# linnanwang/FastGen

Measured on AMD Instinct MI355X. Metric: images/sec at 4-step distilled (DMD2) sampling, higher is better.
Workload: dtype fp32 (tensors, accumulate) with split-bf16 x3 MFMA conv products; 1 GPU; EDM CIFAR-10 32x32 SongUNet (55.7M params) DMD2 4-step 'sde' sampling, batch=512 per GPU; global_batch=512, sample_steps=4, parallelism=replicas x1 (no data-path collective), graph=True

## Files before the change

### fastgen_amd/_lib.py

```python
import ctypes
import os
from ctypes import POINTER, c_char_p, c_double, c_float, c_int, c_int64, c_size_t, c_uint64, c_void_p

_HERE = os.path.dirname(os.path.abspath(__file__))
LIB_PATH = os.path.join(_HERE, "libfastgen_amd.so")

FG_MAX_LEVELS = 8
FG_DTYPE_F32, FG_DTYPE_BF16, FG_DTYPE_BF16X3, FG_DTYPE_FP8 = 0, 1, 2, 3
DTYPE_NAMES = {"fp32": FG_DTYPE_F32, "bf16": FG_DTYPE_BF16, "bf16x3": FG_DTYPE_BF16X3, "fp8": FG_DTYPE_FP8}
FG_SAMPLE_SDE, FG_SAMPLE_ODE = 0, 1
SAMPLE_TYPES = {"sde": FG_SAMPLE_SDE, "ode": FG_SAMPLE_ODE}
FG_LOOP_X0, FG_LOOP_MEANFLOW, FG_LOOP_EULER = 0, 1, 2
LOOP_KINDS = {"x0": FG_LOOP_X0, "meanflow": FG_LOOP_MEANFLOW, "euler": FG_LOOP_EULER}
FG_SCHEDULE_EDM, FG_SCHEDULE_RF = 0, 1
FG_DROP_PRECOND_INPUT, FG_DROP_PRECOND_OUTPUT = 1, 2
FG_BWD_DECODER, FG_BWD_ENCODER, FG_BWD_EMBED = 1, 2, 4
FG_MODEL_SONGUNET, FG_MODEL_DHARIWAL = 0, 1


class fg_edm_config(ctypes.Structure):
    _fields_ = [
        ("img_resolution", c_int), ("img_channels", c_int), ("label_dim", c_int), ("augment_dim", c_int),
        ("model_channels", c_int), ("num_levels", c_int), ("channel_mult", c_int * FG_MAX_LEVELS),
        ("channel_mult_emb", c_int), ("num_blocks", c_int), ("num_attn_resolutions", c_int),
# ... 151 lines not shown
    "fg_wan_bind_param": (c_int, [c_void_p, c_char_p, c_void_p, c_int64]),
    "fg_wan_pack_weights": (c_int, [c_void_p, c_void_p]),
    "fg_wan_pack_group": (c_int, [c_void_p, c_char_p, c_char_p, c_void_p]),
    "fg_wan_workspace_bytes": (c_size_t, [c_void_p, c_int, c_int, c_int, c_int]),
    "fg_wan_clear_caches": (c_int, [c_void_p, c_void_p]),
    "fg_wan_set_text": (c_int, [c_void_p, c_void_p, c_int, c_int, c_void_p, c_size_t, c_void_p]),
    "fg_wan_forward": (c_int, [c_void_p, c_void_p, c_void_p, c_void_p, c_int, c_int, c_int, c_int, c_int, c_int, c_void_p, c_size_t,
                               c_void_p]),
    "fg_wan_forward_block_causal": (c_int, [c_void_p, c_void_p, c_void_p, c_void_p, c_int, c_int, c_int, c_int, c_void_p, c_size_t, c_void_p]),
    "fg_wan_forward_features": (c_int, [c_void_p, c_void_p, c_void_p, c_void_p, c_int, c_int, c_int, c_int, c_int, c_int, c_int, POINTER(c_int),
                                        POINTER(fg_wan_block_taps), c_int, c_void_p, c_void_p, c_void_p, c_size_t, c_void_p]),
    "fg_disc_edm_num_params": (c_int, [c_int]),
    "fg_disc_edm_workspace_bytes": (c_size_t, [c_int, c_int]),
    "fg_disc_edm_run": (c_int, [c_void_p, c_int, c_void_p, c_void_p, c_void_p, c_void_p, c_void_p, c_int, c_void_p, c_size_t, c_void_p]),
    "fg_edm_jvp": (c_int, [c_void_p, c_void_p, c_void_p, c_void_p, c_void_p, c_void_p, c_void_p, c_void_p, c_void_p, c_void_p, c_int,
                           c_void_p, c_size_t, c_void_p]),
    "fg_edm_set_dropout": (c_int, [c_void_p, c_float, c_uint64]),
    "fg_op_dropout_mask": (c_int, [c_void_p, c_int64, c_float, ctypes.c_uint32, c_uint64, c_void_p]),
    "fg_edm_set_augment": (c_int, [c_void_p, c_void_p]),
    "fg_edm_set_training": (c_int, [c_void_p, c_int]),
    "fg_op_images_to_u8": (c_int, [c_void_p, c_void_p, c_int64, c_int, c_int, c_int, c_void_p]),
    "fg_op_randn": (c_int, [c_void_p, c_int64, c_uint64, c_uint64, c_void_p]),
    "fg_op_attention": (c_int, [c_void_p, c_void_p, c_void_p, c_void_p, c_int, c_int, c_int, c_int, c_int, c_void_p]),
    "fg_op_attention_split": (c_int, [c_void_p, c_void_p, c_void_p, c_void_p, c_int, c_int, c_int, c_int, c_int, c_int, c_void_p]),
    "fg_op_attention_plan": (c_int, [c_int, c_int, c_int, c_int, c_int, c_int, c_int, c_int, c_int, POINTER(fg_attention_plan)]),
    "fg_op_attention_ex": (c_int, [c_void_p, c_int, c_int64, c_void_p, c_void_p, c_int, c_int64, c_void_p, c_int, c_int64, c_int, c_int, c_int,
                                   c_int, c_int, c_int, c_int, c_int, c_void_p]),
    "fg_op_gemm_bf16": (c_int, [c_void_p, c_void_p, c_void_p, c_void_p, c_int, c_int, c_int, c_int, c_void_p, c_int, c_int, c_void_p,
                                c_int, c_void_p]),
    "fg_op_quant_rows_fp8": (c_int, [c_int, c_void_p, c_void_p, c_void_p, c_int64, c_int, c_void_p]),
    "fg_op_gemm_fp8": (c_int, [c_void_p, c_void_p, c_void_p, c_void_p, c_int, c_int, c_int, c_int, c_void_p, c_int, c_int, c_void_p,
                               c_int, c_void_p, c_void_p, c_void_p]),
    "fg_op_dit_ln_modulate_fp8": (c_int, [c_void_p, c_void_p, c_int, c_int, c_int, c_void_p, c_void_p, c_int, c_int, c_int, c_void_p]),
    "fg_op_gemm_x3": (c_int, [c_void_p, c_void_p, c_void_p, c_void_p, c_int, c_int, c_int, c_int, c_void_p, c_int, c_int, c_void_p,
                              c_int, c_void_p]),
}

_lib = None


def lib():
    global _lib
    if _lib is None:
        if not os.path.exists(LIB_PATH):
            raise RuntimeError(
                f"{LIB_PATH} not found: build it with `python -c 'import __graft_entry__ as g; g.build()'` "
# ... 19 lines not shown
```

### fastgen_amd/csrc/attn.hip

```cpp
#include <cstdlib>
#include "common.h"
#include "misc.h"

namespace {

template <typename T>
struct PFrag;
template <>
struct PFrag<__bf16> {
    static __device__ __forceinline__ Frag8<__bf16> make(const f32x16& p, int s) {
        Frag8<__bf16> f;
#pragma unroll
        for (int j = 0; j < 8; ++j) f.v[j] = (__bf16)p[8 * s + j];
        return f;
    }
};
template <>
struct PFrag<float> {
    static __device__ __forceinline__ Frag8<float> make(const f32x16& p, int s) {
        Frag8<float> f;
        f.lo = f32x4{p[8 * s + 0], p[8 * s + 1], p[8 * s + 2], p[8 * s + 3]};
        f.hi = f32x4{p[8 * s + 4], p[8 * s + 5], p[8 * s + 6], p[8 * s + 7]};
        return f;
    }
// ... 257 lines not shown
                        mma16(o[d], pf[t * 2 + sub][s2], vf);
                    }
            __syncthreads();
            __builtin_amdgcn_sched_barrier(0);
        }
#pragma unroll
        for (int d = 0; d < 4; ++d)
#pragma unroll
            for (int i = 0; i < 16; ++i) obase[(size_t)acc_row(i, h) * D + (dg * 4 + d) * 32] = (__bf16)o[d][i];
    }
}

constexpr int X3_KP = 272, X3_VP = 136;
constexpr int X3_PLANE = 64 * X3_KP;
constexpr int X3_BUF = 2 * X3_PLANE;

struct AttnMerge {
    const float2* ab;
    const float* bp;
    float2* stats;
    float scale;
};

template <bool MRG>
__global__ __launch_bounds__(256, 2) void attention_x3_lds_kernel(const float* __restrict__ q, const float* __restrict__ k,
                                                                  const float* __restrict__ vt, float* __restrict__ out, int B,
                                                                  AttnMerge mg) {
    constexpr int Tn = 256, D = 256;
    extern __shared__ __attribute__((aligned(16))) char smem[];
    const int tid = threadIdx.x, lane = tid & 63, wave = tid >> 6;
    const int r = lane & 31, h = lane >> 5;
    const int n = blockIdx.x >> 1;
    const int q0 = (blockIdx.x & 1) * 128 + wave * 32;

    auto stage_k = [&](int s, char* buf) {
        const float* src = k + ((size_t)n * Tn + (s & 3) * 64) * D + (s >> 2) * 128;
        f32x4 cf[4];
        if constexpr (MRG) {
            const f32x4* cp = reinterpret_cast<const f32x4*>(mg.ab + (size_t)n * D + (s >> 2) * 128 + (tid & 15) * 8);
#pragma unroll
            for (int j = 0; j < 4; ++j) cf[j] = cp[j];
        }
#pragma unroll
        for (int b2 = 0; b2 < 2; ++b2) {
#pragma unroll
            for (int i = b2 * 2; i < b2 * 2 + 2; ++i) {
                const int idx = tid + 256 * i, row = idx >> 4, c = idx & 15;
                float x[8];
                widen8(load_frag(src + (size_t)row * D + c * 8), x);
                if constexpr (MRG) {
#pragma unroll
                    for (int j = 0; j < 8; ++j) x[j] = fmaf(x[j], cf[j >> 1][2 * (j & 1)], cf[j >> 1][2 * (j & 1) + 1]);
                }
                bf16x8 hi, lo;
                split8(x, hi, lo);
                *reinterpret_cast<bf16x8*>(buf + row * X3_KP + c * 16) = hi;
// ... 4 lines not shown
    };
    auto stage_v = [&](int s, char* buf) {
        const float* src = vt + ((size_t)n * D + (s >> 2) * 128) * Tn + (s & 3) * 64;
#pragma unroll
        for (int b2 = 0; b2 < 2; ++b2) {
#pragma unroll
            for (int i = b2 * 2; i < b2 * 2 + 2; ++i) {
                const int idx = tid + 256 * i, row = idx >> 3, c = idx & 7;
                float x[8];
                widen8(load_frag(src + (size_t)row * Tn + c * 8), x);
                bf16x8 hi, lo;
                split8(x, hi, lo);
                bf16x4* dh = reinterpret_cast<bf16x4*>(buf + row * X3_VP + c * 16);
                dh[0] = bf16x4{hi[0], hi[1], hi[2], hi[3]};
                dh[1] = bf16x4{hi[4], hi[5], hi[6], hi[7]};
                bf16x4* dl = reinterpret_cast<bf16x4*>(buf + X3_PLANE + row * X3_VP + c * 16);
                dl[0] = bf16x4{lo[0], lo[1], lo[2], lo[3]};
                dl[1] = bf16x4{lo[4], lo[5], lo[6], lo[7]};
            }
            __builtin_amdgcn_sched_barrier(0);
        }
    };

    const float* qrow = q + ((size_t)n * Tn + q0 + r) * D + 8 * h;
    f32x16 st[8];
#pragma unroll
    for (int kt = 0; kt < 8; ++kt)
#pragma unroll
        for (int i = 0; i < 16; ++i) st[kt][i] = 0.f;

    stage_k(0, smem);
    __syncthreads();
    Frag8<bf16x3> qf[8];
#pragma unroll
    for (int s = 0; s < 8; ++s) {
        const char* cur = smem + (s & 1) * X3_BUF;
        if ((s & 3) == 0) {
#pragma unroll
            for (int kk = 0; kk < 8; ++kk) qf[kk] = load_op<bf16x3>(qrow + (s >> 2) * 128 + kk * 16);
        }
        if (s + 1 < 8) stage_k(s + 1, smem + ((s + 1) & 1) * X3_BUF);
#pragma unroll
        for (int kk = 0; kk < 8; ++kk) {
#pragma unroll
            for (int sub = 0; sub < 2; ++sub) {
                const char* p = cur + (sub * 32 + r) * X3_KP + (kk * 16 + 8 * h) * 2;
                Frag8<bf16x3> kf;
                kf.hi = *reinterpret_cast<const bf16x8*>(p);
                kf.lo = *reinterpret_cast<const bf16x8*>(p + X3_PLANE);
                mma16(st[(s & 3) * 2 + sub], kf, qf[kk]);
            }
        }
        __syncthreads();
        __builtin_amdgcn_sched_barrier(0);
    }

    float m = -INFINITY;
#pragma unroll
    for (int kt = 0; kt < 8; ++kt)
#pragma unroll
        for (int i = 0; i < 16; ++i) m = fmaxf(m, st[kt][i]);
    m = fmaxf(m, __shfl_xor(m, 32));
    float sum = 0.f;
#pragma unroll
    for (int kt = 0; kt < 8; ++kt)
#pragma unroll
        for (int i = 0; i < 16; ++i) {
            const float e = __builtin_amdgcn_exp2f(1.44269504088896341f * 0.0625f * (st[kt][i] - m));
            st[kt][i] = e;
            sum += e;
        }
    sum += __shfl_xor(sum, 32);
    const float inv = __builtin_amdgcn_rcpf(sum);
    Frag8<bf16x3> pf[8][2];
#pragma unroll
    for (int kt = 0; kt < 8; ++kt) {
#pragma unroll
        for (int s2 = 0; s2 < 2; ++s2) {
            float v[8];
#pragma unroll
            for (int j = 0; j < 8; ++j) v[j] = st[kt][8 * s2 + j] * inv;
            split8(v, pf[kt][s2].hi, pf[kt][s2].lo);
        }
        __builtin_amdgcn_sched_barrier(0);
    }

    float* obase = out + ((size_t)n * Tn + q0) * D + r;
    stage_v(0, smem);
    __syncthreads();
    f32x16 o[4];
#pragma unroll
    for (int s = 0; s < 8; ++s) {
        const char* cur = smem + (s & 1) * X3_BUF;
        if ((s & 3) == 0) {
#pragma unroll
            for (int d = 0; d < 4; ++d)
#pragma unroll
                for (int i = 0; i < 16; ++i) o[d][i] = 0.f;
        }
        if (s + 1 < 8) stage_v(s + 1, smem + ((s + 1) & 1) * X3_BUF);
#pragma unroll
        for (int sub = 0; sub < 2; ++sub)
#pragma unroll
            for (int s2 = 0; s2 < 2; ++s2)
#pragma unroll
                for (int d = 0; d < 4; ++d) {
                    const char* p = cur + (d * 32 + r) * X3_VP + (sub * 32 + 16 * s2 + 4 * h) * 2;
                    const bf16x4 a0 = *reinterpret_cast<const bf16x4*>(p), a1 = *reinterpret_cast<const bf16x4*>(p + 16);
                    const bf16x4 b0 = *reinterpret_cast<const bf16x4*>(p + X3_PLANE), b1 = *reinterpret_cast<const bf16x4*>(p + X3_PLANE + 16);
                    Frag8<bf16x3> vf;
                    vf.hi = bf16x8{a0[0], a0[1], a0[2], a0[3], a1[0], a1[1], a1[2], a1[3]};
                    vf.lo = bf16x8{b0[0], b0[1], b0[2], b0[3], b1[0], b1[1], b1[2], b1[3]};
                    mma16(o[d], pf[(s & 3) * 2 + sub][s2], vf);
                }
        __syncthreads();
        __builtin_amdgcn_sched_barrier(0);
        if ((s & 3) == 3) {
            if constexpr (MRG) {
                const float* xbase = k + ((size_t)n * Tn + q0) * D + r;
#pragma unroll
                for (int d = 0; d < 4; ++d) {
                    const int col = ((s >> 2) * 4 + d) * 32;
                    const float bias = mg.bp[col + r];
                    float sv = 0.f, qv = 0.f;
#pragma unroll
                    for (int i = 0; i < 16; ++i) {
                        const size_t off = (size_t)acc_row(i, h) * D + col;
                        const float v = (o[d][i] + bias + xbase[off]) * mg.scale;
                        obase[off] = v;
                        sv += v;
                        qv += v * v;
                    }
                    if (mg.stats) {
                        sv += __shfl_xor(sv, 32), qv += __shfl_xor(qv, 32);
                        sv += __shfl_xor(sv, 1), qv += __shfl_xor(qv, 1);
                        sv += __shfl_xor(sv, 2), qv += __shfl_xor(qv, 2);
                        if (h == 0 && (r & 3) == 0)
                            mg.stats[((size_t)n * 8 + (blockIdx.x & 1) * 4 + wave) * (D / 4) + ((col + r) >> 2)] = make_float2(sv, qv);
                    }
                }
            } else {
#pragma unroll
                for (int d = 0; d < 4; ++d)
#pragma unroll
                    for (int i = 0; i < 16; ++i) obase[(size_t)acc_row(i, h) * D + ((s >> 2) * 4 + d) * 32] = o[d][i];
            }
        }
    }
}

__global__ void attn_merge_weights_kernel(const float* __restrict__ qkv_w, const float* __restrict__ qkv_b, const float* __restrict__ proj_w,
                                          float* __restrict__ w_out, float* __restrict__ b_out, int C) {
    const int o = blockIdx.x % C;
    const bool val = blockIdx.x >= C;
    for (int i = threadIdx.x; i <= C; i += blockDim.x) {
        double acc = 0.0;
        for (int c = 0; c < C; ++c) {
            const double l = val ? proj_w[(size_t)o * C + c] : qkv_w[(size_t)(3 * c + 1) * C + o];
            const int row = 3 * c + (val ? 2 : 0);
            acc += l * (double)(i < C ? qkv_w[(size_t)row * C + i] : qkv_b[row]);
        }
        if (i < C)
            w_out[(size_t)blockIdx.x * C + i] = (float)acc;
        else
            b_out[blockIdx.x] = (float)acc;
    }
}

template <bool MRG>
int x3_lds_prepare() {
    static bool done[16] = {};
    const int dev = fg_device_slot();
    if (dev < 0) return (int)hipErrorInvalidDevice;
    if (!done[dev]) {
        hipError_t e = hipFuncSetAttribute(reinterpret_cast<const void*>(attention_x3_lds_kernel<MRG>), hipFuncAttributeMaxDynamicSharedMemorySize, 2 * X3_BUF);
        if (e != hipSuccess) return (int)e;
        done[dev] = true;
    }
    return 0;
}

}

int launch_attn_merge_weights(const float* qkv_w, const float* qkv_b, const float* proj_w, float* w_out, float* b_out, int C, hipStream_t s) {
    hipLaunchKernelGGL(attn_merge_weights_kernel, dim3(2 * C), dim3(256), 0, s, qkv_w, qkv_b, proj_w, w_out, b_out, C);
    return (int)hipGetLastError();
}

int launch_attention_merged(const float* qm, const float* x_mid, const float2* ab, const float* vmt, const float* bp, float scale, float* out,
                            float2* stats, int B, hipStream_t s) {
    const int rc = x3_lds_prepare<true>();
    if (rc || !qm) return rc;
    hipLaunchKernelGGL(attention_x3_lds_kernel<true>, dim3(B * 2), dim3(256), 2 * X3_BUF, s, qm, x_mid, vmt, out, B, AttnMerge{ab, bp, stats, scale});
    return (int)hipGetLastError();
}

int launch_attention(int dtype, const void* q, const void* k, const void* vt, void* out, int B, int T, hipStream_t s) {
    if (T != 256 && T != 64) return (int)hipErrorInvalidValue;
    const int nt = T / 32;
    const int waves = B * nt;
    dim3 grid((waves + 3) / 4), block(256);
    if (dtype == 1 && nt == 8) {
        static bool attr_done_dev[16] = {};
        const int dev = fg_device_slot();
        if (dev < 0) return (int)hipErrorInvalidDevice;
        bool& attr_done = attr_done_dev[dev];
        if (!attr_done) {
            hipError_t e = hipFuncSetAttribute(reinterpret_cast<const void*>(attention_lds_kernel), hipFuncAttributeMaxDynamicSharedMemorySize, 2 * ATT_BUF);
            if (e != hipSuccess) return (int)e;
            attr_done = true;
        }
        if (!q) return 0;
        hipLaunchKernelGGL(attention_lds_kernel, dim3(B * 2), block, 2 * ATT_BUF, s, (const __bf16*)q, (const __bf16*)k, (const __bf16*)vt, (__bf16*)out, B);
        return (int)hipGetLastError();
    }
    static const bool x3_lds = [] {
        const char* e = getenv("FASTGEN_AMD_ATTN_X3_LDS");
        return !(e && e[0] == '0');
// ... 28 lines not shown
```

### fastgen_amd/csrc/conv.h

```cpp
#pragma once
#include <hip/hip_runtime.h>

struct ConvArgs {
    const void* src1;
    const void* src2;
    int C1, C2;
    int Hs, Ws;
    int H, W;
    int B;
    const float2* ab;
    const void* wpack;
    const void* wpack_ws;
    const float* bias;
    const float* temb;
    int temb_stride;
    const void* resid;
    int rshift = 0;
    float scale;
    void* out;
    int Cout;
    float2* stats;
    int dbg;
    void* q_out;
    void* k_out;
    void* vt_out;
    const float* gate = nullptr;
    int gate_stride = 0;
    int act = 0;
    int heads = 0, head_dim = 0;
    size_t heads_lo_off = 0;
};

enum { PRO_NONE = 0, PRO_GN = 1, PRO_GN_SILU = 2 };
enum { RES_NONE = 0, RES_DOWN = 1, RES_UP = 2, RES_SUBPIX = 3 };
enum { OUT_NHWC = 0, OUT_QKV = 1, OUT_TOK = 2, OUT_HEADS = 3, OUT_QV = 4 };

int launch_conv_fused(int dtype, int ks, int pro, int res, int outmode, const ConvArgs& a, hipStream_t stream);
int conv_stat_slots(int W);
bool conv_ws_supported(int dtype, int ks, int pro, int res, int outmode, const ConvArgs& a);
bool conv_ws_enabled();
int launch_conv_ws(int res, const ConvArgs& a, hipStream_t stream, bool prepare_only, int pro = PRO_GN_SILU);
bool conv_ws_shape_ok(int dtype, int cout, int cin, int res);
int launch_pack_conv_weights_ws(const float* w_oihw, void* wpack_ws, int cout, int cin, hipStream_t stream);
bool conv_x3ws_supported(int ks, int pro, int res, int outmode, const ConvArgs& a);
bool conv_x3ws_shape_ok(int cout, int cin, int res);
int conv_x3ws_stat_slots(int W, int res);
int launch_conv_x3ws(int res, const ConvArgs& a, hipStream_t stream, bool prepare_only, int pro = PRO_GN_SILU);
int launch_pack_conv_weights_x3ws(const float* w_oihw, void* wpack_ws, int cout, int cin, hipStream_t stream);
// ... 10 lines not shown
```

### fastgen_amd/csrc/conv.hip

```cpp
#include "common.h"
#include "conv.h"
#include <stdlib.h>
#include <string.h>

#include <type_traits>

namespace {

constexpr int PITCH = 144;
constexpr int NTHR = 256;

template <int KS, int LOGW>
struct Geom {
    static constexpr int W = 1 << LOGW;
    static constexpr int LOGTW = (LOGW == 5) ? 4 : LOGW;
    static constexpr int TW = 1 << LOGTW;
    static constexpr int LOGTH = 3;
    static constexpr int TH = 1 << LOGTH;
    static constexpr int IMGS = 128 / (TH * TW);
    static constexpr int TCOLS = W / TW;
    static constexpr int TPI = (IMGS > 1) ? 1 : (W / TH) * TCOLS;
    static constexpr int PAD = KS / 2;
    static constexpr int HW_ = TW + 2 * PAD;
    static constexpr int HH_ = TH + 2 * PAD;
// ... 372 lines not shown
            if (!qk && a.temb && n < a.B) add += *reinterpret_cast<const f32x4*>(a.temb + (size_t)n * a.temb_stride + co0);
            f32x4 gate4 = {1.f, 1.f, 1.f, 1.f};
            if (OUTMODE == OUT_TOK && a.gate && n < a.B) gate4 = *reinterpret_cast<const f32x4*>(a.gate + (size_t)n * a.gate_stride + co0);
#pragma unroll
            for (int j = 0; j < NP; ++j) {
                const int pl = j * RP + prow;
                f32x4 v = *reinterpret_cast<const f32x4*>(ep + pl * EP_PITCH + c4 * 16);
                bool ok;
                const size_t go = goff(mt, j, ok);
                if (ok) {
                    v += add;
                    if (OUTMODE == OUT_TOK) {
                        if (a.act == 1) {
#pragma unroll
                            for (int e = 0; e < 4; ++e) v[e] = gelu_tanh_f(v[e]);
                        }
                        v *= gate4;
                    }
                    if (resid) v += widen4(rcur[j]);
                    v *= a.scale;
                    f32x4 vr;
                    if constexpr (OUTMODE == OUT_HEADS && std::is_same<T, bf16x3>::value) {
                        vr = store4_split(reinterpret_cast<__bf16*>(out) + go, a.heads_lo_off, v);
                    } else {
                        vr = store4(out + go, v);
                    }
                    ssum[im] += (vr[0] + vr[1]) + (vr[2] + vr[3]);
                    ssq[im] += (vr[0] * vr[0] + vr[1] * vr[1]) + (vr[2] * vr[2] + vr[3] * vr[3]);
                }
            }
#pragma unroll
            for (int j = 0; j < NP; ++j) rcur[j] = rnext[j];
        }
        if (!qk && a.stats) {
#pragma unroll
            for (int im = 0; im < G::IMGS; ++im) {
                float sv = ssum[im], qv = ssq[im];
#pragma unroll
                for (int sh = QPW; sh < 64; sh <<= 1) {
                    sv += __shfl_xor(sv, sh);
                    qv += __shfl_xor(qv, sh);
                }
                const int n = n_base + im;
                if (prow == 0 && n < a.B)
                    a.stats[((size_t)n * G::TPI + slot) * (a.Cout >> 2) + (co0 >> 2)] = make_float2(sv, qv);
            }
        }
    } else {
        static_assert(!QKM || NT == 2, "qkv epilogue assumes 64 channels per wave");
        ST* vt = reinterpret_cast<ST*>(a.vt_out);
#pragma unroll
        for (int nt = 0; nt < NT; ++nt) {
            const int cg = nblk * (128 * NT) + wave * (32 * NT) + nt * 32 + r;
            const int cl = (OUTMODE == OUT_HEADS) ? cg - 2 * a.heads * a.head_dim : wave * 64 + nt * 32 + r;
            const float bias = a.bias ? a.bias[OUTMODE == OUT_HEADS ? cg : nblk * 256 + cl] : 0.f;
#pragma unroll
            for (int mt = 0; mt < 4; ++mt) {
#pragma unroll
                for (int i4 = 0; i4 < 16; i4 += 4) {
                    const int p = mt * 32 + acc_row(i4, h);
                    const int x = col0 + (p & (G::TW - 1));
                    const int y = row0 + ((p >> G::LOGTW) & (G::TH - 1));
                    const int n = n_base + (p >> (G::LOGTW + G::LOGTH));
                    if (n < a.B)
                    {
                        const size_t vo = ((size_t)n * (OUTMODE == OUT_HEADS ? a.heads * a.head_dim : 256) + cl) * HWo + y * G::W + x;
                        const f32x4 vv = {acc[mt][nt][i4] + bias, acc[mt][nt][i4 + 1] + bias, acc[mt][nt][i4 + 2] + bias,
                                          acc[mt][nt][i4 + 3] + bias};
                        if constexpr (OUTMODE == OUT_HEADS && std::is_same<T, bf16x3>::value)
                            store4_split(reinterpret_cast<__bf16*>(vt) + vo, a.heads_lo_off, vv);
                        else
                            store4(vt + vo, vv);
                    }
                }
            }
        }
    }
}
// ... 236 lines not shown
```

### fastgen_amd/csrc/engine.hip

```cpp
#include <hip/hip_runtime.h>

#include <cmath>
#include <cstdarg>
#include <cstdio>
#include <cstdlib>
#include <cstring>
#include <string>
#include <map>
#include <vector>

#include "../../include/fastgen_amd.h"
#include "common.h"
#include "adm.h"
#include "edm2.h"
#include "conv.h"
#include "misc.h"

namespace {

thread_local std::string g_err;

int fail(int code, const char* fmt, ...) {
    char buf[512];
    va_list ap;
// ... 765 lines not shown
        HIP_TRY(conv_launch(h, 1, PRO_NONE, low ? RES_NONE : res_mode, OUT_NHWC, k, s));
        resid = w.sbuf;
        d.rshift = low ? 1 : 0;
    }
    HIP_TRY(launch_gn_finalize(w.h.st, b.cout, w.h.slots, nullptr, 0, 0, h->P(b.norm1_w), h->P(b.norm1_b), kBlockEps, w.ab1, B, hw, s, w.mr1));
    Act& x_mid = b.attn ? w.xattn : out;
    d.resid = resid; d.out = x_mid.p; d.stats = x_mid.st;
    if (w.a1d) {
        HIP_TRY(launch_gn_act(h->dtype, 0, w.h.p, b.cout, nullptr, 0, w.ab1, w.a1d, B, b.res_out, 0, s, w.drop));
        d.src1 = w.a1d; d.ab = nullptr;
        x_mid.slots = conv_launch_stat_slots(h->cmode, 3, PRO_NONE, RES_NONE, OUT_NHWC, d);
        HIP_TRY(conv_launch(h, 3, PRO_NONE, RES_NONE, OUT_NHWC, d, s));
    } else {
        x_mid.slots = conv_launch_stat_slots(h->cmode, 3, PRO_GN_SILU, RES_NONE, OUT_NHWC, d);
        HIP_TRY(conv_launch(h, 3, PRO_GN_SILU, RES_NONE, OUT_NHWC, d, s));
    }
    if (b.attn) {
        HIP_TRY(launch_gn_finalize(x_mid.st, b.cout, x_mid.slots, nullptr, 0, 0, h->P(b.norm2_w), h->P(b.norm2_b), kBlockEps, w.ab2, B, hw, s, w.mr2));
        ConvArgs q{};
        q.src1 = x_mid.p; q.C1 = b.cout; q.Hs = q.Ws = q.H = q.W = b.res_out; q.B = B;
        if (w.infer && !w.a1d && h->cmode == FG_DTYPE_BF16X3 && hw == 256 && b.cout == 256 && b.p_qv && attn_merge_enabled()) {
            q.ab = w.ab2; q.wpack = b.p_qv; q.bias = b.qv_bias; q.scale = 1.0f; q.Cout = 2 * b.cout;
            q.q_out = w.q; q.vt_out = w.vt;
            HIP_TRY(conv_launch(h, 1, PRO_GN, RES_NONE, OUT_QV, q, s));
            HIP_TRY(launch_attention_merged((const float*)w.q, (const float*)x_mid.p, w.ab2, (const float*)w.vt, h->P(b.proj_b), kSkipScale,
                                            (float*)out.p, out.st, B, s));
            out.slots = 8;
            return FG_OK;
        }
        q.ab = w.ab2; q.wpack = b.p_qkv; q.bias = b.qkv_bias; q.scale = 1.0f; q.Cout = 3 * b.cout;
        q.q_out = w.q; q.k_out = w.k; q.vt_out = w.vt;
        HIP_TRY(conv_launch(h, 1, PRO_GN, RES_NONE, OUT_QKV, q, s));
        HIP_TRY(launch_attention(h->cmode, w.q, w.k, w.vt, w.aout, B, hw, s));
        ConvArgs p{};
        p.src1 = w.aout; p.C1 = b.cout; p.Hs = p.Ws = p.H = p.W = b.res_out; p.B = B;
        p.wpack = b.p_proj; p.bias = h->P(b.proj_b); p.resid = x_mid.p; p.scale = kSkipScale; p.out = out.p; p.Cout = b.cout;
        p.stats = out.st;
        HIP_TRY(conv_launch(h, 1, PRO_NONE, RES_NONE, OUT_NHWC, p, s));
        out.slots = slots;
    }
    return FG_OK;
}

int run_mapping(fg_edm* h, const float* labels, int B, Workspace& w, hipStream_t s) {
    const fg_edm_config& c = h->cfg;
    HIP_TRY(launch_mapping_in(w.coef + B, w.coef + 4 * (size_t)B, h->freqs, labels, c.label_dim,
                              h->P(h->find("model.map_label.weight")), h->P(h->find("model.map_label.bias")), w.emb0, B,
                              h->cond_ch, h->noise_ch, s, h->augment, h->augment ? h->P(h->find("model.map_augment.weight")) : nullptr, c.augment_dim));
    HIP_TRY(launch_linear(w.emb0, h->P(h->find("model.map_layer0.weight")), h->P(h->find("model.map_layer0.bias")), w.emb1,
// ... 693 lines not shown
    if (p.refusal == FG_FA_REFUSE_PATH)
        return fail(FG_EINVAL, "fg_op_attention: kernel form %d cannot serve head_dim %d, batch %d, heads %d, lq %d, lkv %d, scratch %d, force_split %d",
                    path, head_dim, batch, heads, lq, lkv, use_scratch != 0, force_split);
    if (p.refusal)
        return fail(FG_EINVAL, "fg_op_attention: bad argument (head_dim 128 or 72, counts > 0, ldk %% 8, force_split in [0, 8] and > 1 only with scratch)");
    void* scratch = nullptr;
    if (use_scratch) HIP_TRY(hipMalloc(&scratch, fa128_scratch_bytes(batch, heads, lq)));
    const int rc = launch_fa(head_dim, q, ldq, q_bs, k, v, ldk, kv_bs, out, ldo, o_bs, batch, heads, lq, lkv, (hipStream_t)stream, scratch,
                             force_split, path);
    (void)hipStreamSynchronize((hipStream_t)stream);
    (void)hipFree(scratch);
    HIP_TRY(rc);
    return FG_OK;
}
int fg_op_attention_split(const void* q, const void* k, const void* v, void* out, int batch, int heads, int head_dim, int lq, int lkv, int nsplit,
                          void* stream) {
    if (batch <= 0 || heads <= 0 || lq <= 0 || lkv <= 0 || (head_dim != 128 && head_dim != 72))
        return fail(FG_EINVAL, "fg_op_attention: bad argument (head_dim 128 or 72)");
    if (nsplit < 0 || nsplit > 8) return fail(FG_EINVAL, "fg_op_attention_split: nsplit must be in [0, 8]");
    const int D = heads * head_dim;
    return fg_op_attention_ex(q, D, (int64_t)lq * D, k, v, D, (int64_t)lkv * D, out, D, (int64_t)lq * D, batch, heads, head_dim, lq, lkv, 1, nsplit,
                              0, stream);
}
int fg_op_attention(const void* q, const void* k, const void* v, void* out, int batch, int heads, int head_dim, int lq, int lkv, void* stream) {
    return fg_op_attention_split(q, k, v, out, batch, heads, head_dim, lq, lkv, 0, stream);
}
int fg_op_gemm_bf16(const void* a, const void* w, const float* bias, void* out, int m, int n, int k, int act, const float* gate,
                    int gate_stride, int gate_rows, const void* resid, int tile_order, void* stream) {
#ifdef FG_TIMING_BUILD
    const int act_ok = 1 | 4 | 8, order_ok = 1023;
#else
    const int act_ok = 1, order_ok = 127 | 256 | 512;
#endif
    if (act < 0 || (act & ~act_ok)) return fail(FG_EINVAL, "fg_op_gemm_bf16: act must be 0 (none) or 1 (GELU tanh), got %d", act);
    if (tile_order < 0 || (tile_order & ~order_ok)) return fail(FG_EINVAL, "fg_op_gemm_bf16: bad tile_order %d", tile_order);
    if (((tile_order >> 4) & 1) + ((tile_order >> 5) & 1) + ((tile_order >> 8) & 1) + ((tile_order >> 9) & 1) > 1)
        return fail(FG_EINVAL, "fg_op_gemm_bf16: tile_order bits 16, 32, 256 and 512 exclude each other");
    GemmArgs g;
    g.A = a; g.W = w; g.bias = bias; g.out = out; g.M = m; g.N = n; g.K = k; g.act = act;
    g.gate = gate; g.gate_stride = gate_stride; g.gate_rows = gate_rows > 0 ? gate_rows : 1; g.resid = resid; g.xn = tile_order & 15;
    g.variant = (tile_order & 16) ? 0 : (tile_order & 32) ? 1 : (tile_order & 256) ? 2 : (tile_order & 512) ? 3 : -1;
    if (!gemm_bf16_supported(g)) return fail(FG_EINVAL, "fg_op_gemm_bf16: unsupported shape (k %% 64, n %% 16, pointers)");
    HIP_TRY(launch_gemm_bf16(g, (hipStream_t)stream, true));
    void* scratch = nullptr;
    hipError_t herr = hipSuccess;
#ifdef FG_TIMING_BUILD
// ... 107 lines not shown
```

### fastgen_amd/csrc/misc.h

```cpp
#pragma once
#include <hip/hip_runtime.h>
#include <stdint.h>

int launch_gn_coeffs(int dtype, const void* x1, int c1, const void* x2, int c2, const float* gamma, const float* beta,
                     float eps, float2* ab, int batch, int hw, hipStream_t s, float2* mr = nullptr);
int launch_gn_finalize(const float2* st1, int c1, int s1, const float2* st2, int c2, int s2, const float* gamma,
                       const float* beta, float eps, float2* ab, int batch, int hw, hipStream_t s, float2* mr = nullptr);
int launch_precond_coef(const double* t, int t_stride, const double* r, int r_stride, double sigma_data,
                        double sigma_shift, double clamp_min, int drop, float* coef, int B, hipStream_t s);
int launch_mapping_in(const float* c_noise, const float* r_noise, const float* freqs, const float* labels, int label_dim,
                      const float* wl, const float* bl, float* out, int B, int N, int noise_ch, hipStream_t s, const float* aug = nullptr, const float* wa = nullptr, int aug_dim = 0);
int launch_linear(const float* x, const float* w, const float* bias, float* y, int B, int I, int O, int act_silu,
                  hipStream_t s);
int launch_conv_in(int dtype, const float* x, const float* c_in, const float* w, const float* bias, void* out, int B,
                   int res, int cin, int cout, hipStream_t s);
int launch_aux_out(int dtype, const void* x, const float2* ab, const float* w, const float* bias, const float* x_t,
                   const float* coef, float* out, int B, int res, int C, int cout, hipStream_t s, float* raw = nullptr);
int launch_latents(const float* noise, double tv, const double* tp, int ti, float* out, int64_t total, hipStream_t s);
int launch_forward_process(const float* x0, const float* eps, double tv, const double* tp, int ti, int sched, float* out,
                           int64_t total, hipStream_t s);
int launch_x0_to_eps(const float* xt, const float* x0, double tv, const double* tp, int ti, int sched, double clamp_min,
                     float* out, int64_t total, hipStream_t s);
int launch_meanflow_update(const float* x, const float* u, const double* tp, int ia, int ib, float* out, int64_t total,
                           hipStream_t s);
// ... 53 lines not shown
int launch_attention_jvp(int dtype, const void* q, const void* k, const void* vt, const void* qd, const void* kd, const void* vtd, void* od,
                         void* scratch, int B, int T, int C, hipStream_t s);
size_t attention_backward_scratch_bytes(int dtype, int B, int T, int C);
int launch_attention_backward(int dtype, const void* q, const void* k, const void* vt, const void* dO, void* dq, void* dk, void* dvt,
                              void* scratch, int B, int T, int C, hipStream_t s);
int launch_qkv_interleave(int dtype, const void* dq, const void* dk, const void* dvt, void* out, int B, int T, int C, hipStream_t s);
int launch_nt_gemm(const void* A, const void* Bm, void* C, int M, int N, int K, float scale, int out_bf16, hipStream_t s);
int launch_transpose_bf16(const void* in, void* out, int R, int Cc, hipStream_t s);
int disc_num_params(int res);
size_t disc_workspace_bytes(int res, int B);
int disc_run(const float* feat, int res, const float* const* params, float* logits, const float* dlogits, float* dfeat,
             float* const* grads, int B, void* ws, hipStream_t s);
int conv_wgrad_supported(int res, int cin, int cout, int ks);
size_t conv_wgrad_workspace_bytes(int B, int res, int cin, int cout, int ks);
int launch_conv_wgrad(int mode, const void* act, const void* dy, float* dw, int B, int res, int cin, int cout, int ks, int accumulate,
                      void* workspace, hipStream_t s, float scale = 1.0f);
int launch_images_to_u8(const float* x, uint8_t* out, int64_t B, int C, int HW, hipStream_t s);
int launch_act_to_nchw(int dtype, const void* in, float* out, int B, int C, int HW, hipStream_t s);
int launch_nchw_to_nhwc(const float* in, float* out, int B, int C, int HW, hipStream_t s);

int launch_attention(int dtype, const void* q, const void* k, const void* vt, void* out, int B, int T, hipStream_t s);
int launch_attn_merge_weights(const float* qkv_w, const float* qkv_b, const float* proj_w, float* w_out, float* b_out, int C, hipStream_t s);
int launch_attention_merged(const float* qm, const float* x_mid, const float2* ab, const float* vmt, const float* bp, float scale, float* out,
                            float2* stats, int B, hipStream_t s);

size_t aux_pack_elems(int C);
int launch_pack_aux_weights(int dtype, const float* w, void* out, int C, int cout, hipStream_t s);
int aux_head_supported(int dtype, int res, int C, int cout);
int launch_aux_head(int dtype, const void* x, const float2* ab, const void* wpack, const float* bias, const float* x_t,
                    const float* coef, float* out, int B, int C, int cout, hipStream_t s, float* raw = nullptr);

int stem_supported(int res, int cin, int cout);
size_t stem_pack_elems();
int launch_pack_stem_weights(int dtype, const float* w, void* out, int cin, hipStream_t s);
int launch_stem(int dtype, const float* x, const float* c_in, const void* wpack, const float* bias, void* out, float2* stats,
                int B, int res, int cin, hipStream_t s);

int launch_dit_ln_modulate(int dtype, int D, const void* x, const float* mod, int mod_stride, int shift_off, int scale_off, void* y,
                           int ntok, int tokens_per_image, hipStream_t s);
int launch_dit_ln_modulate_split(int D, const float* x, const float* mod, int mod_stride, int shift_off, int scale_off, void* y, int ntok,
                                 int tokens_per_image, hipStream_t s);
int launch_dit_ln_modulate_fp8(int D, const void* x, const float* mod, int mod_stride, int shift_off, int scale_off, void* y, float* y_scale,
                               int ntok, int tokens_per_image, hipStream_t s);
int launch_dit_final(int dtype, int D, const void* x, const float* mod, const float* w, const float* bias, float* out, int ntok, int grid,
                     int p, int C, hipStream_t s);
int launch_dit_patch_embed(int dtype, const float* x, const float* w, const float* bias, const float* pos, void* out, int B, int C, int grid,
                           int p, int D, hipStream_t s);
// ... 62 lines not shown
```

### include/fastgen_amd.h

```cpp
#ifndef FASTGEN_AMD_H
#define FASTGEN_AMD_H

#include <stddef.h>
#include <stdint.h>

#ifdef __cplusplus
extern "C" {
#endif

#define FG_API __attribute__((visibility("default")))

#define FG_OK 0
#define FG_EINVAL 1
#define FG_ENOTREADY 2
#define FG_EHIP 3
#define FG_ENOMEM 4

#define FG_DTYPE_F32 0
#define FG_DTYPE_BF16 1
#define FG_DTYPE_BF16X3 2
#define FG_DTYPE_FP8 3

#define FG_SAMPLE_SDE 0
#define FG_SAMPLE_ODE 1
// ... 259 lines not shown
                                 int nsplit, void* stream);
#define FG_FA_TILE128 1
#define FG_FA_TILE128_W3 2
#define FG_FA_TILE128_REG 3
#define FG_FA_WIDE 4
#define FG_FA_WIDE_CUT 5
#define FG_FA_SEQ72 6
#define FG_FA_TILE72 7
#define FG_FA_TILE72_W3 8
#define FG_FA_REFUSE_ARG 1
#define FG_FA_REFUSE_OFFSET 2
#define FG_FA_REFUSE_PATH 3
typedef struct fg_attention_plan {
    int kernel;
    int nsplit;
    int t_cut;
    int sample_major;
    int refusal;
    int64_t grid;
    size_t scratch_bytes;
} fg_attention_plan;
FG_API int fg_op_attention_plan(int head_dim, int batch, int heads, int lq, int lkv, int ldk, int use_scratch, int force_split, int path,
                                fg_attention_plan* plan);
FG_API int fg_op_attention_ex(const void* q, int ldq, int64_t q_bs, const void* k, const void* v, int ldk, int64_t kv_bs, void* out, int ldo,
                              int64_t o_bs, int batch, int heads, int head_dim, int lq, int lkv, int use_scratch, int force_split, int path,
                              void* stream);
FG_API int fg_op_gemm_bf16(const void* a, const void* w, const float* bias, void* out, int m, int n, int k, int act, const float* gate,
                           int gate_stride, int gate_rows, const void* resid, int tile_order, void* stream);
FG_API int fg_op_quant_rows_fp8(int dtype, const void* x, void* q, float* scale, int64_t m, int k, void* stream);
FG_API int fg_op_gemm_fp8(const void* a, const void* w, const float* bias, void* out, int m, int n, int k, int act, const float* gate,
                          int gate_stride, int gate_rows, const void* resid, int tile_order, const float* a_scale, const float* w_scale,
                          void* stream);
FG_API int fg_op_dit_ln_modulate_fp8(const void* x, const float* mod, int mod_stride, int shift_off, int scale_off, void* y, float* y_scale,
                                     int ntok, int d, int tokens_per_image, void* stream);
FG_API int fg_op_gemm_x3(const float* a, const float* w, const float* bias, void* out, int m, int n, int k, int act, const float* gate,
                         int gate_stride, int gate_rows, const float* resid, int out_mode, void* stream);

typedef struct fg_edm2_config {
    int img_resolution;
    int img_channels;
    int label_dim;
    int model_channels;
    int num_levels;
    int channel_mult[FG_MAX_LEVELS];
    int channel_mult_noise;
    int channel_mult_emb;
// ... 40 lines not shown
```

Before: 2881 img/s.

## Emit pre-split bf16 Q/V planes from QV conv and DMA V into LDS

The merged-attention QV conv can now write Q and transposed V as pre-split bf16 hi/lo planes, so the attention kernel no longer re-splits fp32 values. A new attention kernel variant loads Q directly as planes, streams V into swizzled LDS with buffer-load-to-LDS DMA, software-pipelines the K staging around the MFMA loop, and remaps workgroups across XCDs. This removes split arithmetic and register staging for V and aims to overlap global loads with compute. It is on by default via an env flag and adds LDS for cached affine coefficients, which may affect occupancy.

```diff
diff --git a/fastgen_amd/_lib.py b/fastgen_amd/_lib.py
--- a/fastgen_amd/_lib.py
+++ b/fastgen_amd/_lib.py
@@ -197,6 +197,7 @@
     "fg_op_images_to_u8": (c_int, [c_void_p, c_void_p, c_int64, c_int, c_int, c_int, c_void_p]),
     "fg_op_randn": (c_int, [c_void_p, c_int64, c_uint64, c_uint64, c_void_p]),
     "fg_op_attention": (c_int, [c_void_p, c_void_p, c_void_p, c_void_p, c_int, c_int, c_int, c_int, c_int, c_void_p]),
+    "fg_op_attn_wg_map": (c_int, [c_int, c_int]),
     "fg_op_attention_split": (c_int, [c_void_p, c_void_p, c_void_p, c_void_p, c_int, c_int, c_int, c_int, c_int, c_int, c_void_p]),
     "fg_op_attention_plan": (c_int, [c_int, c_int, c_int, c_int, c_int, c_int, c_int, c_int, c_int, POINTER(fg_attention_plan)]),
     "fg_op_attention_ex": (c_int, [c_void_p, c_int, c_int64, c_void_p, c_void_p, c_int, c_int64, c_void_p, c_int, c_int64, c_int, c_int, c_int,
diff --git a/fastgen_amd/csrc/attn.hip b/fastgen_amd/csrc/attn.hip
--- a/fastgen_amd/csrc/attn.hip
+++ b/fastgen_amd/csrc/attn.hip
@@ -303,16 +303,20 @@
     float scale;
 };
 
-template <bool MRG>
+__host__ __device__ inline int attn_wg_map(int b, int grid) { return (grid & 7) ? b : (b & 7) * (grid >> 3) + (b >> 3); }
+
+template <bool MRG, bool PL = false>
 __global__ __launch_bounds__(256, 2) void attention_x3_lds_kernel(const float* __restrict__ q, const float* __restrict__ k,
                                                                   const float* __restrict__ vt, float* __restrict__ out, int B,
                                                                   AttnMerge mg) {
+    static_assert(MRG || !PL, "the planes come from the merged block's OUT_QV conv");
     constexpr int Tn = 256, D = 256;
     extern __shared__ __attribute__((aligned(16))) char smem[];
     const int tid = threadIdx.x, lane = tid & 63, wave = tid >> 6;
     const int r = lane & 31, h = lane >> 5;
-    const int n = blockIdx.x >> 1;
-    const int q0 = (blockIdx.x & 1) * 128 + wave * 32;
+    const int bid = PL ? attn_wg_map((int)blockIdx.x, (int)gridDim.x) : (int)blockIdx.x;
+    const int n = bid >> 1;
+    const int q0 = (bid & 1) * 128 + wave * 32;
 
     auto stage_k = [&](int s, char* buf) {
         const float* src = k + ((size_t)n * Tn + (s & 3) * 64) * D + (s >> 2) * 128;
@@ -363,14 +367,78 @@
         }
     };
 
+    __amdgpu_buffer_rsrc_t rsX, rsQ, rsO;
+    if constexpr (PL) {
+        rsX = __builtin_amdgcn_make_buffer_rsrc(const_cast<float*>(k) + (size_t)n * Tn * D, 0, Tn * D * 4, 0x00020000);
+        rsQ = __builtin_amdgcn_make_buffer_rsrc(const_cast<float*>(q) + (size_t)n * Tn * D, 0, Tn * D * 4, 0x00020000);
+        rsO = __builtin_amdgcn_make_buffer_rsrc(out + (size_t)n * Tn * D, 0, Tn * D * 4, 0x00020000);
+    }
+    const int ko = ((tid >> 4) * D + (tid & 15) * 8) * 4;
+    auto load_k = [&](int s, int half, Frag8<float> (&kr)[2]) {
+#pragma unroll
+        for (int i = 0; i < 2; ++i) {
+            const int so = (((s & 3) * 64 + 16 * (2 * half + i)) * D + (s >> 2) * 128) * 4;
+            kr[i].lo = __builtin_bit_cast(f32x4, __builtin_amdgcn_raw_buffer_load_b128(rsX, ko, so, 0));
+            kr[i].hi = __builtin_bit_cast(f32x4, __builtin_amdgcn_raw_buffer_load_b128(rsX, ko + 16, so, 0));
+        }
+    };
+    auto put_k = [&](int s, int half, const Frag8<float> (&kr)[2], char* buf) {
+        const f32x4* cp = reinterpret_cast<const f32x4*>(smem + 2 * X3_BUF) + (s >> 2) * 64 + (tid & 15) * 4;
+        f32x4 cf[4];
+#pragma unroll
+        for (int j = 0; j < 4; ++j) cf[j] = cp[j];
+#pragma unroll
+        for (int i = 0; i < 2; ++i) {
+            const int idx = tid + 256 * (2 * half + i), row = idx >> 4, c = idx & 15;
+            float x[8];
+            widen8(kr[i], x);
+#pragma unroll
+            for (int j = 0; j < 8; ++j) x[j] = fmaf(x[j], cf[j >> 1][2 * (j & 1)], cf[j >> 1][2 * (j & 1) + 1]);
+            bf16x8 hi, lo;
+            split8(x, hi, lo);
+            *reinterpret_cast<bf16x8*>(buf + row * X3_KP + c * 16) = hi;
+            *reinterpret_cast<bf16x8*>(buf + X3_PLANE + row * X3_KP + c * 16) = lo;
+        }
+    };
+    typedef __attribute__((address_space(3))) void* lds_ptr;
+    __amdgpu_buffer_rsrc_t rsV;
+    unsigned vvo[2] = {0, 0};
+    if constexpr (PL) {
+        rsV = __builtin_amdgcn_make_buffer_rsrc(const_cast<float*>(vt) + (size_t)n * D * Tn, 0, D * Tn * 4, 0x00020000);
+#pragma unroll
+        for (int jp = 0; jp < 2; ++jp) {
+            const int row = (wave & 1) * 64 + jp * 8 + (lane >> 3);
+            vvo[jp] = (unsigned)(row * 1024 + (wave >> 1) * 512 + (((lane & 7) ^ ((row >> 1) & 7)) * 16));
+        }
+    }
+    auto dma_v = [&](int s, char* buf) {
+        const int so = (s >> 2) * (128 * 1024) + (s & 3) * 128;
+#pragma unroll
+        for (int j = 0; j < 8; ++j)
+            __builtin_amdgcn_raw_ptr_buffer_load_lds(rsV, (lds_ptr)(buf + (wave >> 1) * X3_PLANE + ((wave & 1) * 8 + j) * 1024), 16, vvo[j & 1],
+                                                     so + (j >> 1) * 16384, 0, 0);
+    };
+    const int vsw = (h ^ ((r >> 1) & 7)) * 16;
+
     const float* qrow = q + ((size_t)n * Tn + q0 + r) * D + 8 * h;
+    const int qo = ((q0 + r) * D + 8 * h) * 4;
     f32x16 st[8];
 #pragma unroll
     for (int kt = 0; kt < 8; ++kt)
 #pragma unroll
         for (int i = 0; i < 16; ++i) st[kt][i] = 0.f;
 
-    stage_k(0, smem);
+    Frag8<float> kr[2];
+    if constexpr (PL) {
+        load_k(0, 0, kr);
+        reinterpret_cast<float2*>(smem + 2 * X3_BUF)[tid] = mg.ab[(size_t)n * D + tid];
+        __syncthreads();
+        put_k(0, 0, kr, smem);
+        load_k(0, 1, kr);
+        put_k(0, 1, kr, smem);
+    } else {
+        stage_k(0, smem);
+    }
     __syncthreads();
     Frag8<bf16x3> qf[8];
 #pragma unroll
@@ -378,11 +446,33 @@
         const char* cur = smem + (s & 1) * X3_BUF;
         if ((s & 3) == 0) {
 #pragma unroll
-            for (int kk = 0; kk < 8; ++kk) qf[kk] = load_op<bf16x3>(qrow + (s >> 2) * 128 + kk * 16);
-        }
-        if (s + 1 < 8) stage_k(s + 1, smem + ((s + 1) & 1) * X3_BUF);
+            for (int kk = 0; kk < 8; ++kk) {
+                if constexpr (PL) {
+                    const bf16x8 q0v = __builtin_bit_cast(bf16x8, __builtin_amdgcn_raw_buffer_load_b128(rsQ, qo, ((s >> 2) * 128 + kk * 16) * 4, 0));
+                    const bf16x8 q1v = __builtin_bit_cast(bf16x8, __builtin_amdgcn_raw_buffer_load_b128(rsQ, qo + 16, ((s >> 2) * 128 + kk * 16) * 4, 0));
+                    qf[kk].hi = bf16x8{q0v[0], q0v[1], q0v[2], q0v[3], q1v[0], q1v[1], q1v[2], q1v[3]};
+                    qf[kk].lo = bf16x8{q0v[4], q0v[5], q0v[6], q0v[7], q1v[4], q1v[5], q1v[6], q1v[7]};
+                } else {
+                    qf[kk] = load_op<bf16x3>(qrow + (s >> 2) * 128 + kk * 16);
+                }
+            }
+        }
+        if constexpr (PL) {
+            if (s + 1 < 8) load_k(s + 1, 0, kr);
+            __builtin_amdgcn_sched_barrier(0);
+        } else {
+            if (s + 1 < 8) stage_k(s + 1, smem + ((s + 1) & 1) * X3_BUF);
+        }
 #pragma unroll
         for (int kk = 0; kk < 8; ++kk) {
+            if constexpr (PL) {
+                if (kk == 4 && s + 1 < 8) {
+                    __builtin_amdgcn_sched_barrier(0);
+                    put_k(s + 1, 0, kr, smem + ((s + 1) & 1) * X3_BUF);
+                    load_k(s + 1, 1, kr);
+                    __builtin_amdgcn_sched_barrier(0);
+                }
+            }
 #pragma unroll
             for (int sub = 0; sub < 2; ++sub) {
                 const char* p = cur + (sub * 32 + r) * X3_KP + (kk * 16 + 8 * h) * 2;
@@ -392,10 +482,15 @@
                 mma16(st[(s & 3) * 2 + sub], kf, qf[kk]);
             }
         }
+        if constexpr (PL) {
+            __builtin_amdgcn_sched_barrier(0);
+            if (s + 1 < 8) put_k(s + 1, 1, kr, smem + ((s + 1) & 1) * X3_BUF);
+        }
         __syncthreads();
         __builtin_amdgcn_sched_barrier(0);
     }
 
+    if constexpr (PL) dma_v(0, smem);
     float m = -INFINITY;
 #pragma unroll
     for (int kt = 0; kt < 8; ++kt)
@@ -427,7 +522,10 @@
     }
 
     float* obase = out + ((size_t)n * Tn + q0) * D + r;
-    stage_v(0, smem);
+    if constexpr (PL)
+        asm volatile("s_waitcnt vmcnt(0)" ::: "memory");
+    else
+        stage_v(0, smem);
     __syncthreads();
     f32x16 o[4];
 #pragma unroll
@@ -439,25 +537,63 @@
 #pragma unroll
                 for (int i = 0; i < 16; ++i) o[d][i] = 0.f;
         }
-        if (s + 1 < 8) stage_v(s + 1, smem + ((s + 1) & 1) * X3_BUF);
+        if constexpr (PL) {
+            if (s + 1 < 8) dma_v(s + 1, smem + ((s + 1) & 1) * X3_BUF);
+            __builtin_amdgcn_sched_barrier(0);
+        } else {
+            if (s + 1 < 8) stage_v(s + 1, smem + ((s + 1) & 1) * X3_BUF);
+        }
 #pragma unroll
         for (int sub = 0; sub < 2; ++sub)
 #pragma unroll
             for (int s2 = 0; s2 < 2; ++s2)
 #pragma unroll
                 for (int d = 0; d < 4; ++d) {
-                    const char* p = cur + (d * 32 + r) * X3_VP + (sub * 32 + 16 * s2 + 4 * h) * 2;
-                    const bf16x4 a0 = *reinterpret_cast<const bf16x4*>(p), a1 = *reinterpret_cast<const bf16x4*>(p + 16);
-                    const bf16x4 b0 = *reinterpret_cast<const bf16x4*>(p + X3_PLANE), b1 = *reinterpret_cast<const bf16x4*>(p + X3_PLANE + 16);
                     Frag8<bf16x3> vf;
-                    vf.hi = bf16x8{a0[0], a0[1], a0[2], a0[3], a1[0], a1[1], a1[2], a1[3]};
-                    vf.lo = bf16x8{b0[0], b0[1], b0[2], b0[3], b1[0], b1[1], b1[2], b1[3]};
+                    if constexpr (PL) {
+                        const char* p = cur + (d * 32 + r) * 128 + (((sub * 2 + s2) * 32) ^ vsw);
+                        vf.hi = *reinterpret_cast<const bf16x8*>(p);
+                        vf.lo = *reinterpret_cast<const bf16x8*>(p + X3_PLANE);
+                    } else {
+                        const char* p = cur + (d * 32 + r) * X3_VP + (sub * 32 + 16 * s2 + 4 * h) * 2;
+                        const bf16x4 a0 = *reinterpret_cast<const bf16x4*>(p), a1 = *reinterpret_cast<const bf16x4*>(p + 16);
+                        const bf16x4 b0 = *reinterpret_cast<const bf16x4*>(p + X3_PLANE), b1 = *reinterpret_cast<const bf16x4*>(p + X3_PLANE + 16);
+                        vf.hi = bf16x8{a0[0], a0[1], a0[2], a0[3], a1[0], a1[1], a1[2], a1[3]};
+                        vf.lo = bf16x8{b0[0], b0[1], b0[2], b0[3], b1[0], b1[1], b1[2], b1[3]};
+                    }
                     mma16(o[d], pf[(s & 3) * 2 + sub][s2], vf);
                 }
+        if constexpr (PL) asm volatile("s_waitcnt vmcnt(0)" ::: "memory");
         __syncthreads();
         __builtin_amdgcn_sched_barrier(0);
         if ((s & 3) == 3) {
-            if constexpr (MRG) {
+            if constexpr (PL) {
+                const int eo = ((q0 + 4 * h) * D + r) * 4;
+#pragma unroll
+                for (int d = 0; d < 4; ++d) {
+                    const int col = ((s >> 2) * 4 + d) * 32;
+                    const float bias = mg.bp[col + r];
+                    float xr[16];
+#pragma unroll
+                    for (int i = 0; i < 16; ++i)
+                        xr[i] = __builtin_bit_cast(float, __builtin_amdgcn_raw_buffer_load_b32(rsX, eo, (acc_row(i, 0) * D + col) * 4, 0));
+                    float sv = 0.f, qv = 0.f;
+#pragma unroll
+                    for (int i = 0; i < 16; ++i) {
+                        const float v = (o[d][i] + bias + xr[i]) * mg.scale;
+                        __builtin_amdgcn_raw_buffer_store_b32(__builtin_bit_cast(unsigned, v), rsO, eo, (acc_row(i, 0) * D + col) * 4, 0);
+                        sv += v;
+                        qv += v * v;
+                    }
+                    if (mg.stats) {
+                        sv += __shfl_xor(sv, 32), qv += __shfl_xor(qv, 32);
+                        sv += __shfl_xor(sv, 1), qv += __shfl_xor(qv, 1);
+                        sv += __shfl_xor(sv, 2), qv += __shfl_xor(qv, 2);
+                        if (h == 0 && (r & 3) == 0)
+                            mg.stats[((size_t)n * 8 + (bid & 1) * 4 + wave) * (D / 4) + ((col + r) >> 2)] = make_float2(sv, qv);
+                    }
+                }
+            } else if constexpr (MRG) {
                 const float* xbase = k + ((size_t)n * Tn + q0) * D + r;
 #pragma unroll
                 for (int d = 0; d < 4; ++d) {
@@ -477,7 +613,7 @@
                         sv += __shfl_xor(sv, 1), qv += __shfl_xor(qv, 1);
                         sv += __shfl_xor(sv, 2), qv += __shfl_xor(qv, 2);
                         if (h == 0 && (r & 3) == 0)
-                            mg.stats[((size_t)n * 8 + (blockIdx.x & 1) * 4 + wave) * (D / 4) + ((col + r) >> 2)] = make_float2(sv, qv);
+                            mg.stats[((size_t)n * 8 + (bid & 1) * 4 + wave) * (D / 4) + ((col + r) >> 2)] = make_float2(sv, qv);
                     }
                 }
             } else {
@@ -486,6 +622,7 @@
 #pragma unroll
                     for (int i = 0; i < 16; ++i) obase[(size_t)acc_row(i, h) * D + ((s >> 2) * 4 + d) * 32] = o[d][i];
             }
+            if constexpr (PL) __builtin_amdgcn_sched_barrier(0);
         }
     }
 }
@@ -508,13 +645,15 @@
     }
 }
 
-template <bool MRG>
+constexpr int X3_AB = 256 * 8;
+template <bool MRG, bool PL = false>
 int x3_lds_prepare() {
     static bool done[16] = {};
     const int dev = fg_device_slot();
     if (dev < 0) return (int)hipErrorInvalidDevice;
     if (!done[dev]) {
-        hipError_t e = hipFuncSetAttribute(reinterpret_cast<const void*>(attention_x3_lds_kernel<MRG>), hipFuncAttributeMaxDynamicSharedMemorySize, 2 * X3_BUF);
+        hipError_t e = hipFuncSetAttribute(reinterpret_cast<const void*>(attention_x3_lds_kernel<MRG, PL>), hipFuncAttributeMaxDynamicSharedMemorySize,
+                                           2 * X3_BUF + (PL ? X3_AB : 0));
         if (e != hipSuccess) return (int)e;
         done[dev] = true;
     }
@@ -529,12 +668,26 @@
 }
 
 int launch_attention_merged(const float* qm, const float* x_mid, const float2* ab, const float* vmt, const float* bp, float scale, float* out,
-                            float2* stats, int B, hipStream_t s) {
-    const int rc = x3_lds_prepare<true>();
+                            float2* stats, int B, hipStream_t s, bool planes) {
+    int rc = x3_lds_prepare<true>();
+    if (!rc) rc = x3_lds_prepare<true, true>();
     if (rc || !qm) return rc;
-    hipLaunchKernelGGL(attention_x3_lds_kernel<true>, dim3(B * 2), dim3(256), 2 * X3_BUF, s, qm, x_mid, vmt, out, B, AttnMerge{ab, bp, stats, scale});
+    if (planes)
+        hipLaunchKernelGGL((attention_x3_lds_kernel<true, true>), dim3(B * 2), dim3(256), 2 * X3_BUF + X3_AB, s, qm, x_mid, vmt, out, B,
+                           AttnMerge{ab, bp, stats, scale});
+    else
+        hipLaunchKernelGGL(attention_x3_lds_kernel<true>, dim3(B * 2), dim3(256), 2 * X3_BUF, s, qm, x_mid, vmt, out, B, AttnMerge{ab, bp, stats, scale});
     return (int)hipGetLastError();
 }
+
+bool attn_planes_enabled() {
+    static const bool on = [] {
+        const char* e = getenv("FASTGEN_AMD_ATTN_PLANES");
+        return !(e && e[0] == '0');
+    }();
+    return on;
+}
+int attn_wg_map_host(int grid, int block) { return attn_wg_map(block, grid); }
 
 int launch_attention(int dtype, const void* q, const void* k, const void* vt, void* out, int B, int T, hipStream_t s) {
     if (T != 256 && T != 64) return (int)hipErrorInvalidValue;
diff --git a/fastgen_amd/csrc/conv.h b/fastgen_amd/csrc/conv.h
--- a/fastgen_amd/csrc/conv.h
+++ b/fastgen_amd/csrc/conv.h
@@ -24,6 +24,7 @@
     void* q_out;
     void* k_out;
     void* vt_out;
+    int qv_planes = 0;
     const float* gate = nullptr;
     int gate_stride = 0;
     int act = 0;
diff --git a/fastgen_amd/csrc/conv.hip b/fastgen_amd/csrc/conv.hip
--- a/fastgen_amd/csrc/conv.hip
+++ b/fastgen_amd/csrc/conv.hip
@@ -418,6 +418,19 @@
                     f32x4 vr;
                     if constexpr (OUTMODE == OUT_HEADS && std::is_same<T, bf16x3>::value) {
                         vr = store4_split(reinterpret_cast<__bf16*>(out) + go, a.heads_lo_off, v);
+                    } else if constexpr (OUTMODE == OUT_QV) {
+                        if (a.qv_planes) {
+                            bf16x4 qh, ql;
+#pragma unroll
+                            for (int e = 0; e < 4; ++e) {
+                                qh[e] = (__bf16)v[e];
+                                ql[e] = (__bf16)(v[e] - (float)qh[e]);
+                            }
+                            *reinterpret_cast<bf16x8*>(out + go) = bf16x8{qh[0], qh[1], qh[2], qh[3], ql[0], ql[1], ql[2], ql[3]};
+                            vr = v;
+                        } else {
+                            vr = store4(out + go, v);
+                        }
                     } else {
                         vr = store4(out + go, v);
                     }
@@ -450,6 +463,29 @@
             const int cg = nblk * (128 * NT) + wave * (32 * NT) + nt * 32 + r;
             const int cl = (OUTMODE == OUT_HEADS) ? cg - 2 * a.heads * a.head_dim : wave * 64 + nt * 32 + r;
             const float bias = a.bias ? a.bias[OUTMODE == OUT_HEADS ? cg : nblk * 256 + cl] : 0.f;
+            if (OUTMODE == OUT_QV && a.qv_planes) {
+                static_assert(OUTMODE != OUT_QV || (G::W == 16 && G::TW == 16), "the key order is that of a 16-wide image row");
+#pragma unroll
+                for (int mt = 0; mt < 4; ++mt) {
+#pragma unroll
+                    for (int i8 = 0; i8 < 16; i8 += 8) {
+                        const int p = mt * 32 + acc_row(i8, h);
+                        const int y = row0 + ((p >> G::LOGTW) & (G::TH - 1));
+                        const int n = n_base + (p >> (G::LOGTW + G::LOGTH));
+                        if (n < a.B) {
+                            float xx[8];
+#pragma unroll
+                            for (int e = 0; e < 8; ++e) xx[e] = acc[mt][nt][i8 + e] + bias;
+                            bf16x8 vh, vl;
+                            split8(xx, vh, vl);
+                            __bf16* d = reinterpret_cast<__bf16*>(vt) + ((size_t)n * 256 + cl) * 512 + y * 16 + 8 * h;
+                            *reinterpret_cast<bf16x8*>(d) = vh;
+                            *reinterpret_cast<bf16x8*>(d + 256) = vl;
+                        }
+                    }
+                }
+                continue;
+            }
 #pragma unroll
             for (int mt = 0; mt < 4; ++mt) {
 #pragma unroll
diff --git a/fastgen_amd/csrc/engine.hip b/fastgen_amd/csrc/engine.hip
--- a/fastgen_amd/csrc/engine.hip
+++ b/fastgen_amd/csrc/engine.hip
@@ -811,9 +811,10 @@
         if (w.infer && !w.a1d && h->cmode == FG_DTYPE_BF16X3 && hw == 256 && b.cout == 256 && b.p_qv && attn_merge_enabled()) {
             q.ab = w.ab2; q.wpack = b.p_qv; q.bias = b.qv_bias; q.scale = 1.0f; q.Cout = 2 * b.cout;
             q.q_out = w.q; q.vt_out = w.vt;
+            q.qv_planes = attn_planes_enabled();
             HIP_TRY(conv_launch(h, 1, PRO_GN, RES_NONE, OUT_QV, q, s));
             HIP_TRY(launch_attention_merged((const float*)w.q, (const float*)x_mid.p, w.ab2, (const float*)w.vt, h->P(b.proj_b), kSkipScale,
-                                            (float*)out.p, out.st, B, s));
+                                            (float*)out.p, out.st, B, s, q.qv_planes != 0));
             out.slots = 8;
             return FG_OK;
         }
@@ -1553,6 +1554,7 @@
     return fg_op_attention_ex(q, D, (int64_t)lq * D, k, v, D, (int64_t)lkv * D, out, D, (int64_t)lq * D, batch, heads, head_dim, lq, lkv, 1, nsplit,
                               0, stream);
 }
+int fg_op_attn_wg_map(int grid, int block) { return (grid <= 0 || block < 0 || block >= grid) ? -1 : attn_wg_map_host(grid, block); }
 int fg_op_attention(const void* q, const void* k, const void* v, void* out, int batch, int heads, int head_dim, int lq, int lkv, void* stream) {
     return fg_op_attention_split(q, k, v, out, batch, heads, head_dim, lq, lkv, 0, stream);
 }
diff --git a/fastgen_amd/csrc/misc.h b/fastgen_amd/csrc/misc.h
--- a/fastgen_amd/csrc/misc.h
+++ b/fastgen_amd/csrc/misc.h
@@ -99,7 +99,9 @@
 int launch_attention(int dtype, const void* q, const void* k, const void* vt, void* out, int B, int T, hipStream_t s);
 int launch_attn_merge_weights(const float* qkv_w, const float* qkv_b, const float* proj_w, float* w_out, float* b_out, int C, hipStream_t s);
 int launch_attention_merged(const float* qm, const float* x_mid, const float2* ab, const float* vmt, const float* bp, float scale, float* out,
-                            float2* stats, int B, hipStream_t s);
+                            float2* stats, int B, hipStream_t s, bool planes = false);
+bool attn_planes_enabled();
+int attn_wg_map_host(int grid, int block);
 
 size_t aux_pack_elems(int C);
 int launch_pack_aux_weights(int dtype, const float* w, void* out, int C, int cout, hipStream_t s);
diff --git a/include/fastgen_amd.h b/include/fastgen_amd.h
--- a/include/fastgen_amd.h
+++ b/include/fastgen_amd.h
@@ -305,6 +305,7 @@
 } fg_attention_plan;
 FG_API int fg_op_attention_plan(int head_dim, int batch, int heads, int lq, int lkv, int ldk, int use_scratch, int force_split, int path,
                                 fg_attention_plan* plan);
+FG_API int fg_op_attn_wg_map(int grid, int block);
 FG_API int fg_op_attention_ex(const void* q, int ldq, int64_t q_bs, const void* k, const void* v, int ldk, int64_t kv_bs, void* out, int ldo,
                               int64_t o_bs, int batch, int heads, int head_dim, int lq, int lkv, int use_scratch, int force_split, int path,
                               void* stream);
```

After: 2896 img/s, median of 6. No clear change (+0.5%).
